# Nablax/Path-Tracer-CUDA-OpenGL

Hardware: AMD Instinct MI355X
Metric: Mray/s + ms/frame, bunny-in-Cornell 1920×1080 @1024spp, 1/2/4/8 MI355X (higher is better)
Workload: dtype f32

## Files before the change

path-tracer-cuda-opengl_amd/csrc/pt_device.hip:

```cpp
#include <hip/hip_runtime.h>

#include <algorithm>
#include <array>
#include <atomic>
#include <chrono>
#include <cfloat>
#include <cmath>
#include <cstdio>
#include <cstdlib>
#include <cstring>
#include <limits>
#include <type_traits>
#include <memory>
#include <string>
#include <vector>

#include "../host/pt_error.hpp"
#include "../host/pt_host.hpp"
#include "../host/pt_inst_dev.hpp"
#include "../host/pt_instancing.hpp"
#include "../host/pt_wide8.hpp"
#include "../host/pt_wide_dev.hpp"
#include "pt.h"
#include "pt_math.hpp"

using pt::fail;

#include "pt_prims.hpp"

namespace pt {
int launchCompatWide(int stack, const void* params, hipStream_t st);
int compatWideWavesPerCU(int stack, int& n);
}

#define HIP_TRY(expr)                                                                        \
    do {                                                                                     \
        hipError_t _e = (expr);                                                              \
        if (_e != hipSuccess)                                                                \
            return fail(PT_ERR_HIP, std::string(#expr) + ": " + hipGetErrorString(_e));      \
    } while (0)

namespace {

constexpr int kWave = 64;
constexpr uint32_t kLeafBit = 0x80000000u;
constexpr uint32_t kSphereBit = 0x40000000u;
constexpr uint32_t kPrimMask = 0x3fffffffu;
constexpr int kJumpMats = 32;
constexpr int kNumCounters = 32;

struct DevScene {
    const float4* nodes;
    const float4* prims;
    const float4* shade;
    const float4* mats;
// ... 293 lines not shown
    const float3 s1 = cross3(d, e2);
    const float det = dot3(s1, e1);
    const float3 s = sub(o, v0);
    const float3 s2 = cross3(s, e1);
    const float inv = rcpRNWave(det, hasM);
    const float t = dot3(s2, e2) * inv;
    const float b1 = dot3(s1, s) * inv;
    const float b2 = dot3(s2, d) * inv;
    const int k = (int)__float_as_uint(q.p0.w);
    const uint64_t rejM = __ballot(b1 >= 1.0f) | __ballot(b1 <= 0.0f) | __ballot(b2 >= 1.0f) | __ballot(b2 <= 0.0f) |
                          __ballot(b1 + b2 >= 1.0f);
    const uint64_t hitM = hasM & __ballot(det != 0.0f) & __ballot(t > tmin) & ~rejM;
    const uint64_t takeM = hitM & (__ballot(t < closest) | (__ballot(t == closest) & __ballot(k < best)));
    const float mid = __builtin_amdgcn_fmed3f(t, closest, t2);
    t2 = __builtin_amdgcn_inverse_ballot_w64(hitM) ? mid : t2;
    closest = __builtin_amdgcn_inverse_ballot_w64(takeM) ? t : closest;
    best = __builtin_amdgcn_inverse_ballot_w64(takeM) ? k : best;
}
__device__ __forceinline__ bool deferredRedo(float4 xy, float2 z, float3 o, float3 inv, float closest, float t2) {
    const SlabHit b = slabPair(v2f{xy.x, xy.y}, v2f{xy.z, xy.w}, v2f{z.x, z.y}, o, inv, 0.001f, __builtin_inff());
    return !b.hit || (closest < b.lo && t2 < b.lo);
}

template <bool MIX = false>
__device__ __forceinline__ uint32_t wideHits(uint4 n0, uint4 n1, uint4 n2, uint4 n3, uint4 n4, float3 o, float3 inv,
                                             uint32_t oct, float tmin, float tmax) {
    constexpr uint32_t kMixExp = MIX ? 24u : 0u;
    const float ax = __uint_as_float(((n0.w & 0xffu) + kMixExp) << 23) * inv.x;
    const float ay = __uint_as_float((((n0.w >> 8) & 0xffu) + kMixExp) << 23) * inv.y;
    const float az = __uint_as_float((((n0.w >> 16) & 0xffu) + kMixExp) << 23) * inv.z;
    const float bx = (__uint_as_float(n0.x) - o.x) * inv.x;
    const float by = (__uint_as_float(n0.y) - o.y) * inv.y;
    const float bz = (__uint_as_float(n0.z) - o.z) * inv.z;
    const bool sx = inv.x < 0.0f, sy = inv.y < 0.0f, sz = inv.z < 0.0f;
    const uint32_t nearX[2] = {sx ? n2.z : n2.x, sx ? n2.w : n2.y}, farX[2] = {sx ? n2.x : n2.z, sx ? n2.y : n2.w};
    const uint32_t nearY[2] = {sy ? n3.z : n3.x, sy ? n3.w : n3.y}, farY[2] = {sy ? n3.x : n3.z, sy ? n3.y : n3.w};
    const uint32_t nearZ[2] = {sz ? n4.z : n4.x, sz ? n4.w : n4.y}, farZ[2] = {sz ? n4.x : n4.z, sz ? n4.y : n4.w};
    uint32_t hits = 0u;
#pragma unroll
    for (int h = 0; h < 2; h++) {
        const uint32_t meta4 = h ? n1.w : n1.z;
        const uint32_t inner4 = __builtin_amdgcn_bitop3_b32(meta4, meta4 << 1, 0x10101010u, 0x80);
        const uint32_t inner1 = inner4 >> 4;
        const uint32_t bitIndex4 = (meta4 ^ mulHalves(inner1, oct)) & 0x1f1f1f1fu;
        uint32_t childBits4 = (meta4 >> 5) & 0x07070707u;
        asm("" : "+v"(childBits4));
#pragma unroll
        for (int j = 0; j < 4; j++) {
            float tnx, tny, tnz, tfx, tfy, tfz;
            if constexpr (MIX) {
                const bool hi = (j & 2) != 0;
                const uint32_t px = hi ? planePairHi(nearX[h]) : planePairLo(nearX[h]);
                const uint32_t py = hi ? planePairHi(nearY[h]) : planePairLo(nearY[h]);
// ... 467 lines not shown
    unsigned* taskCounter;
    uint32_t* stackSpill;
    uint32_t ntasks;
    int nwaves;
    uint32_t seed0, seed1;
    uint32_t sampleBase;
    int measureCost;
    int camFar;
    int rawOut;
    int stripeShift, blockShift;
    int splitTiles, splitWays;
    int compatGrid;
    int nCrit, critLanes, critWaves;
    const uint32_t* critList;
    const uint8_t* critFlag;
    uint32_t* pixRays;
    float3 skyH, skyZ;
    int lit;
    const float4* lights;
    int nLights;
    int mis;
    const uint32_t* lightSlot;
    const uint32_t* instLightFirst;
};
template <bool LIT>
__device__ __forceinline__ float3 skyOf(const RenderParams& P, float3 d, float3 att) {
    if constexpr (LIT) return sky(d, att, P.skyH, P.skyZ);
    else return sky(d, att);
}

#ifndef PT_CRIT_PIXELS
#define PT_CRIT_PIXELS 256
#endif
#ifndef PT_CRIT_LANES
#define PT_CRIT_LANES 4
#endif
constexpr int kCritPixels = PT_CRIT_PIXELS;
constexpr int kCritLanes = PT_CRIT_LANES;
__host__ __device__ constexpr bool critFor(bool sample, bool wide, bool inst, int stack) {
    return !sample && wide && !inst && stack <= 8;
}
__device__ __forceinline__ void addBlock(unsigned long long* acc, float3 sum, uint32_t rays, bool cost) {
    const bool small = sum.x >= 0.0f && sum.y >= 0.0f && sum.z >= 0.0f &&
                       fmaxf(fmaxf(sum.x, sum.y), sum.z) < 16777216.0f;
    unsigned long long fx, fy, fz;
    if (__ballot(!small) == 0) {
// ... 227 lines not shown
typedef const __attribute__((address_space(4))) uint32_t* KU32;
__device__ __forceinline__ float3 ld3(const __attribute__((address_space(4))) float3& v) {
    KFloat* f = (KFloat*)&v;
    return f3(f[0], f[1], f[2]);
}
__device__ __forceinline__ DevScene ldScene(KArgs k) {
    DevScene S;
    S.nodes = k->S.nodes; S.prims = k->S.prims; S.shade = k->S.shade; S.mats = k->S.mats;
    S.wnodes = k->S.wnodes; S.wprims = k->S.wprims; S.wshade = k->S.wshade; S.wbox = k->S.wbox; S.rankOf = k->S.rankOf;
    S.iparent = k->S.iparent; S.err = k->S.err; S.nprims = k->S.nprims;
    S.hasSpheres = k->S.hasSpheres;
    S.cx = k->S.cx; S.cy = k->S.cy; S.cz = k->S.cz; S.ext = k->S.ext;
    S.mixLim = k->S.mixLim;
    S.winst = k->S.winst; S.gBits = k->S.gBits;
    return S;
}

template <bool LIT>
__device__ __forceinline__ float3 skyK(float3 d, float3 att) {
    if constexpr (LIT) return sky(d, att, ld3(kargs()->skyH), ld3(kargs()->skyZ));
    else return sky(d, att);
}

template <int STACK, bool SAMPLE, bool WIDE, bool INST = false, bool LIT = false, bool NEE = false, bool MIS = false>
__global__ __launch_bounds__(kWave) __attribute__((amdgpu_waves_per_eu(kWavesPerEU<STACK, SAMPLE, WIDE> - (NEE && STACK >= 16 ? 1 : 0)))) void renderKernelWF(RenderParams P) {
    static_assert(!NEE || (WIDE && LIT), "NEE: the wide kernels' LIT instantiations only");
    static_assert(!MIS || NEE, "MIS: the NEE instantiations only");
    constexpr int LS = kLdsStack<STACK, SAMPLE, WIDE>;
    __shared__ uint32_t stk[LS * kWave];
    constexpr int SPECN = WIDE && !INST ? PT_WIDE_SPEC : 0;
    constexpr bool SPEC = SPECN > 0;
    __shared__ uint32_t pend[SPEC ? 2 * SPECN * kWave : 1];
    __shared__ float wray[INST ? 6 * kWave : 1];
    __shared__ uint4 taskState[SAMPLE ? kWave : 1];
    __shared__ float neeV[NEE ? (MIS ? 10 : 9) * kWave : 1];
    __shared__ uint32_t neeF[NEE ? kWave : 1];
    const int lane = threadIdx.x;
    int bidT = (int)blockIdx.x, slice = -1;
    constexpr bool CRITK = critFor(SAMPLE, WIDE, INST, STACK);
    const bool crit = CRITK && bidT < P.critWaves;
    if constexpr (CRITK) {
        if (!crit) bidT -= P.critWaves;
    }
    if constexpr (!SAMPLE) {
        const int ks = P.splitTiles * P.splitWays;
        if (crit) {
        } else if (bidT < ks) { slice = bidT % P.splitWays; bidT /= P.splitWays; }
        else bidT -= ks - P.splitTiles;
    }
    int tile = (SAMPLE || crit) ? -1 : tileOf(P, bidT), nSamples = SAMPLE ? 0 : P.spp;
// ... 63 lines not shown


#define PT_BEGIN_RAY(SH)                                                                            \
    do {                                                                                          \
        const bool sh_ = NEE && (SH);                                                             \
        if constexpr (NEE) depthLeft -= sh_ ? 0 : 1;                                              \
        else depthLeft--;                                                                         \
        if constexpr (SAMPLE) {    \
            if (kargs()->measureCost)                                                             \
                __hip_atomic_fetch_add(&taskState[lane].w, 1u, __ATOMIC_RELAXED, __HIP_MEMORY_SCOPE_WORKGROUP); \
        }                                                                                         \
        closest = sh_ ? kShadowTmax : __builtin_inff();                                           \
        best = -1;                                                                                \
        sp = 0;                                                                                   \
        qn = 0;                                                                                   \
        if constexpr (CRITK) pxRays++;                                                            \
        if constexpr (WIDE) {                 \
            inv = f3(rcpRN(d.x), rcpRN(d.y), rcpRN(d.z));                                         \
            const uint32_t oc_ = (inv.x < 0.0f ? 1u : 0u) | (inv.y < 0.0f ? 2u : 0u) | (inv.z < 0.0f ? 4u : 0u); \
            oct = oc_;                                                                            \
            tg = 0u;                                                                              \
                    \
                   \
            bestLo = INST || kargs()->S.hasSpheres ? -__builtin_inff() : closest;                  \
            ng = S.nprims > 0 ? (1u << oc_) : 0u;                                                 \
                 \
            if (!INST && ((kargs()->camFar && !sh_ && depthLeft + 1 == kargs()->max_depth) ||      \
                          (PT_WIDE_MIX && mixUnsafe(inv, kargs()->S.mixLim)))) {                   \
                ng = 0u;             \
                oct |= 8u;      \
            }                                                                                     \
            if (INST && kargs()->camFar && !sh_ && depthLeft + 1 == kargs()->max_depth) {          \
                     \
                const auto& K_ = *kargs();                                                        \
                (void)instEntry(K_.S.cx, K_.S.cy, K_.S.cz, K_.S.ext, o, d, inv);                   \
            }                                                                                     \
            if (CRITK && crit) PT_CRIT_TRACE();                                                    \
        } else if (S.nprims <= 1) {                                                               \
            node = -1;                                                                            \
            if (S.nprims == 1) {        \
                const float t1 = primHitT(loadPrim(S, 0), __float_as_uint(S.prims[2].w) != 0, o, d, \
                                          0.001f, closest);                                       \
                if (t1 >= 0.0f) { closest = t1; best = 0; }                                       \
            }                                                                                     \
        } else {                                                                                  \
            inv = f3(rcpRN(d.x), rcpRN(d.y), rcpRN(d.z));                                         \
            node = 0;                                                                             \
        }                                                                                         \
    } while (0)
#define PT_CRIT_TRACE()                                                                             \
    do {                                                                                          \
        const bool lb_ = S.nprims > 1;                                                            \
        const bool sph_ = kargs()->S.hasSpheres != 0;                                             \
        bool redo_ = false;                                                                       \
        for (;;) {                                                                                \
            while (tg) {                                                                          \
                const uint32_t k_ = tgBase + (uint32_t)__builtin_ctz(tg);                         \
                tg &= tg - 1u;                                                                    \
                const float4* w_ = reinterpret_cast<const float4*>(reinterpret_cast<const char*>(S.wprims) + mul48(k_)); \
                const Prim q_{w_[0], w_[1], w_[2]};                                               \
                const bool isS_ = __float_as_uint(q_.p2.w) != 0u;                                 \
                sTris += (uint32_t)__popcll(__ballot(!isS_));                                     \
                sSph += (uint32_t)__popcll(__ballot(isS_));                                       \
                if (sph_) wideTest<true>(q_, o, d, inv, 0.001f, closest, best, bestLo, lb_, redo_, 0u); \
                else if (INST) wideTest<false>(q_, o, d, inv, 0.001f, closest, best, bestLo, lb_, redo_, 0u); \
                else wideTestTri(q_, __ballot(true), o, d, 0.001f, closest, best, bestLo);    \
            }                                                                                     \
            if ((ng & 0xffu) == 0u) {                                                             \
                if (sp == 0) break;                                                               \
                sp--;                                                                             \
                ng = my[sp * kWave];                                                              \
            }                                                                                     \
            const uint32_t bit_ = (uint32_t)__builtin_ctz(ng & 0xffu);                            \
            const uint32_t child_ = (ng >> 8) + (bit_ ^ (oct & 7u));                              \
            ng &= ~(1u << bit_);                                                                  \
            if (ng & 0xffu) { my[sp * kWave] = ng; sp++; }    \
            sVisits += (uint32_t)__popcll(__ballot(true));                                        \
            const uint32_t off_ = mul80(child_);                                                  \
            const uint4 n0_ = __builtin_bit_cast(uint4, __builtin_amdgcn_raw_buffer_load_b128(nodeRsrc, off_, 0, 0)); \
            const uint4 n1_ = __builtin_bit_cast(uint4, __builtin_amdgcn_raw_buffer_load_b128(nodeRsrc, off_ + 16u, 0, 0)); \
            const uint4 n2_ = __builtin_bit_cast(uint4, __builtin_amdgcn_raw_buffer_load_b128(nodeRsrc, off_ + 32u, 0, 0)); \
            const uint4 n3_ = __builtin_bit_cast(uint4, __builtin_amdgcn_raw_buffer_load_b128(nodeRsrc, off_ + 48u, 0, 0)); \
            const uint4 n4_ = __builtin_bit_cast(uint4, __builtin_amdgcn_raw_buffer_load_b128(nodeRsrc, off_ + 64u, 0, 0)); \
            const uint32_t h_ = wideHits<PT_WIDE_MIX != 0>(n0_, n1_, n2_, n3_, n4_, o, inv, oct & 7u, 0.001f, closest); \
            ng = (n1_.x << 8) | (h_ >> 24);                                                      \
            tgBase = n1_.y;                                                                       \
            tg = h_ & 0xffffffu;                                                                  \
        }                                                                                         \
        if (redo_) oct |= 8u;              \
// ... 223 lines not shown
                        tg = hits & 0xffffffu;
                    }
                }
            } else if constexpr (WIDE) {
                if (wantNode) {
                    if (SPEC && laneOf(mL)) {
                        const uint32_t c = SPECN == 1 ? 0u : (oct >> 4) & 3u;
                        pend[(2u * c) * kWave + lane] = tgBase;
                        pend[(2u * c + 1u) * kWave + lane] = tg;
                        oct += 16u;
                    }
                    if constexpr (SPEC) asm volatile("" ::: "memory");
                    if ((ng & 0xffu) == 0u) { sp--; ng = my[sp * kWave]; }
                    const uint32_t bit = (uint32_t)__builtin_ctz(ng & 0xffu);
                    const uint32_t child = (ng >> 8) + (bit ^ (oct & 7u));
                    ng &= ~(1u << bit);
                    if (ng & 0xffu) { my[sp * kWave] = ng; sp++; }
                    const uint32_t off = mul80(child);
                    const uint4 n0 = __builtin_bit_cast(uint4, __builtin_amdgcn_raw_buffer_load_b128(nodeRsrc, off, 0, 0));
                    const uint4 n1 = __builtin_bit_cast(uint4, __builtin_amdgcn_raw_buffer_load_b128(nodeRsrc, off + 16u, 0, 0));
                    const uint4 n2 = __builtin_bit_cast(uint4, __builtin_amdgcn_raw_buffer_load_b128(nodeRsrc, off + 32u, 0, 0));
                    const uint4 n3 = __builtin_bit_cast(uint4, __builtin_amdgcn_raw_buffer_load_b128(nodeRsrc, off + 48u, 0, 0));
                    const uint4 n4 = __builtin_bit_cast(uint4, __builtin_amdgcn_raw_buffer_load_b128(nodeRsrc, off + 64u, 0, 0));
                    const uint32_t hits = wideHits<PT_WIDE_MIX != 0>(n0, n1, n2, n3, n4, o, inv, oct & 7u, 0.001f, closest);
                    ng = (n1.x << 8) | (hits >> 24);
                    tgBase = n1.y;
                    tg = hits & 0xffffffu;
#ifdef PT_DIAG
                    oct &= ~64u;
#endif
                    if (SPEC && tg == 0u && (oct & 48u)) {
                        oct -= 16u;
                        const uint32_t c = SPECN == 1 ? 0u : (oct >> 4) & 3u;
                        tgBase = pend[(2u * c) * kWave + lane];
                        tg = pend[(2u * c + 1u) * kWave + lane];
#ifdef PT_DIAG
                        oct |= 64u;
#endif
                    }
                }
            } else if (wantNode) {
                const uint32_t off = (uint32_t)node * 64u;
                const float4 a = bload4(nodeRsrc, off), b = bload4(nodeRsrc, off + 16u);
                const float4 q = bload4(nodeRsrc, off + 32u), r = bload4(nodeRsrc, off + 48u);
                const uint32_t lref = __float_as_uint(r.x), rref = __float_as_uint(r.y);
                SlabHit2 h2 = slabBoth(a, b, q, o, inv, 0.001f, closest);
                asm volatile("" : "+v"(h2.r.lo));
// ... 49 lines not shown
            if constexpr (WIDE) {
                PT_DIAG_ADD(sPops, (uint32_t)nL);
                uint32_t k0 = 0u, k1 = 0u;
                const bool h0 = laneOf(mL);
                if (h0) k0 = tgBase + (uint32_t)__builtin_ctz(tg);
                tg &= tg - 1u;
                const uint64_t m1 = __ballot((int)tg > 0);
                const bool h1 = laneOf(m1);
                if (h1) k1 = tgBase + (uint32_t)__builtin_ctz(tg);
                tg &= tg - 1u;
                const float4* w0 = reinterpret_cast<const float4*>(reinterpret_cast<const char*>(S.wprims) + mul48(k0));
                const float4* w1 = reinterpret_cast<const float4*>(reinterpret_cast<const char*>(S.wprims) + mul48(k1));
                const Prim q0{w0[0], w0[1], w0[2]}, q1{w1[0], w1[1], w1[2]};
                bool redo = false;
#ifdef PT_DIAG
                {
                    sHalf += (unsigned long long)__popcll(__ballot(h0 && !h1));
                    const bool pk = !INST && (oct & 64u) != 0u;
                    sParkT += (unsigned long long)(__popcll(__ballot(pk && h0)) + __popcll(__ballot(pk && h1)));
                }
#endif
                const bool lb = !INST && S.nprims > 1;
                const uint32_t kh = INST ? (oct >> 8) << kargs()->S.gBits : 0u;
                if (kargs()->S.hasSpheres) {
                    if (h0) wideTest<true>(q0, o, d, inv, 0.001f, closest, best, bestLo, lb, redo, kh);
                    if (h1) wideTest<true>(q1, o, d, inv, 0.001f, closest, best, bestLo, lb, redo, kh);
                    const uint64_t s0 = mL & __ballot(__float_as_uint(q0.p2.w) != 0u);
                    const uint64_t s1 = m1 & __ballot(__float_as_uint(q1.p2.w) != 0u);
                    sTris += (uint32_t)nL + (uint32_t)__popcll(m1) - (uint32_t)__popcll(s0) - (uint32_t)__popcll(s1);
                    sSph += (uint32_t)__popcll(s0) + (uint32_t)__popcll(s1);
                } else {
                    if constexpr (INST) {
                        if (h0) wideTest<false>(q0, o, d, inv, 0.001f, closest, best, bestLo, lb, redo, kh);
                        if (h1) wideTest<false>(q1, o, d, inv, 0.001f, closest, best, bestLo, lb, redo, kh);
                    } else {
                        wideTestTri(q0, mL, o, d, 0.001f, closest, best, bestLo);
                        wideTestTri(q1, m1, o, d, 0.001f, closest, best, bestLo);
                    }
                    sTris += (uint32_t)nL + (uint32_t)__popcll(m1);
                }
                if (redo) oct |= 8u;
                if (SPEC && tg == 0u && (oct & 48u)) {
                    oct -= 16u;
                    const uint32_t c = SPECN == 1 ? 0u : (oct >> 4) & 3u;
                    tgBase = pend[(2u * c) * kWave + lane];
                    tg = pend[(2u * c + 1u) * kWave + lane];
#ifdef PT_DIAG
// ... 24 lines not shown
                    {
                        tested = true;
                        const float t = primHitT(pr, sph, o, d, 0.001f, closest);
                        if (t >= 0.0f) { closest = t; best = (int)k; }
                    }
                }
            }
            sTris += (uint32_t)__popcll(__ballot(tested && !sph));
            sSph += (uint32_t)__popcll(__ballot(tested && sph));
            }
            }
        }
        if (kind == 2) {
            const uint64_t shadeM = mS & ~needTaskM;
            const bool shading = laneOf(shadeM);
            uint32_t nf = 0u;
            if constexpr (NEE) nf = neeF[lane];
            const bool shadowQ = NEE && (nf & 1u) != 0u;
            if constexpr (WIDE && !INST) {
                bool redo = shading && (oct & 8u);
#ifdef PT_DIAG
                bool missed = false;
#endif
                if (!kargs()->S.hasSpheres && S.nprims > 1) {
                    if (shading && best >= 0 && !redo) {
                        const float4* bx = kargs()->S.wbox + 2 * (size_t)best;
                        redo = deferredRedo(bx[0], *reinterpret_cast<const float2*>(bx + 1), o, inv, closest, bestLo);
#ifdef PT_DIAG
                        {
                            const float2 bz_ = *reinterpret_cast<const float2*>(bx + 1);
                            const float4 bx_ = bx[0];
                            missed = !slabPair(v2f{bx_.x, bx_.y}, v2f{bx_.z, bx_.w}, v2f{bz_.x, bz_.y}, o, inv, 0.001f,
                                               __builtin_inff()).hit;
                        }
#endif
                    }
                }
                PT_DIAG_ADD(sRedo, (uint32_t)__popcll(__ballot(redo)));
                PT_DIAG_ADD(sRedoMiss, (uint32_t)__popcll(__ballot(missed)));
                if (redo) {
                    const DevScene S2 = ldScene(kargs());
                    closest = shadowQ ? kShadowTmax : __builtin_inff();
                    const int k = traceRefStackless(S2, o, d, 0.001f, closest);
                    best = k >= 0 ? (int)S2.rankOf[k] : -1;
                }
            }
            PT_DIAG_ADD(itS, 1u);
// ... 154 lines not shown
        atomicAdd(P.counters + 18, cycNp);
        atomicAdd(P.counters + 19, cycBr);
        atomicAdd(P.counters + 20, (unsigned long long)sRedo);
        atomicAdd(P.counters + 21, sSpecN);
        atomicAdd(P.counters + 22, sIdleN);
        atomicAdd(P.counters + 23, (unsigned long long)sRedoMiss);
        atomicAdd(P.counters + 25, sHalf);
        atomicAdd(P.counters + 27, sParkT);
#endif
    }
}
#undef PT_BEGIN_RAY
#undef PT_CRIT_TRACE
#undef PT_NEW_PATH
#undef PT_SKY
#undef PT_TAKE_TASKS
#undef PT_FINISH_TASK
#undef PT_DIAG_ADD

#ifdef PT_TU_COMPAT
}

namespace pt {
int launchCompatWide(int stack, const void* params, hipStream_t st) {
    const RenderParams& P = *static_cast<const RenderParams*>(params);
    const int grid = P.compatGrid;
    switch (stack) {
#define PT_COMPAT_WIDE(S)                                                                    \
        case S:                                                                                  \
            if (P.nLights > 0 && P.mis) renderKernelWF<S, false, true, false, true, true, true><<<grid, kWave, 0, st>>>(P); \
            else if (P.nLights > 0) renderKernelWF<S, false, true, false, true, true><<<grid, kWave, 0, st>>>(P); \
            else if (P.lit) renderKernelWF<S, false, true, false, true><<<grid, kWave, 0, st>>>(P); \
            else renderKernelWF<S, false, true><<<grid, kWave, 0, st>>>(P);                      \
            break;
        PT_COMPAT_WIDE(8)
        PT_COMPAT_WIDE(16)
        PT_COMPAT_WIDE(24)
#undef PT_COMPAT_WIDE
        default: return -1;
    }
    return 0;
}
int compatWideWavesPerCU(int stack, int& n) {
    const void* k = stack == 8 ? reinterpret_cast<const void*>(&renderKernelWF<8, false, true>)
                  : stack == 16 ? reinterpret_cast<const void*>(&renderKernelWF<16, false, true>)
                  : stack == 24 ? reinterpret_cast<const void*>(&renderKernelWF<24, false, true>) : nullptr;
    if (!k || hipOccupancyMaxActiveBlocksPerMultiprocessor(&n, k, kWave, 0) != hipSuccess) return -1;
    return 0;
}
}
#else

__global__ __launch_bounds__(256) void resolveKernel(const float* __restrict__ src,
                                                     const unsigned long long* __restrict__ pixAcc, float* accum,
                                                     float inv, int format, void* out, int64_t npix,
                                                     unsigned* tileCost, int width, int tilesX, int costMax) {
    const int64_t i = (int64_t)blockIdx.x * blockDim.x + threadIdx.x;
    if (i >= npix) return;
    float x, y, z;
    if (!pixAcc) {
        x = src[3 * i + 0]; y = src[3 * i + 1]; z = src[3 * i + 2];
    } else {
        const ulonglong2* a2 = reinterpret_cast<const ulonglong2*>(pixAcc + 4 * i);
        const ulonglong2 a = a2[0], b = a2[1];
        x = fixedToFloat(a.x);
        y = fixedToFloat(a.y);
        z = fixedToFloat(b.x);
        const uint32_t rays = (uint32_t)min(b.y, 0xffffffffull);
        if (tileCost) {
// ... 1275 lines not shown
    s->wideDepth = topDepth + 1 + s->instMaxDepthB + 1;
    s->wideSource = 4;
    s->wideReady = true;
    s->instLights = lights;
    s->nLights = lights ? s->instLightTotal : 0;
    s->buildMs = (double)ms;
    s->wideBuildMs = std::chrono::duration<double, std::milli>(std::chrono::steady_clock::now() - t0).count();
    s->depth = 0;
    if (wideStackFor(s->wideDepth) < 0) return fail(PT_ERR_STATE, "instanced BVH too deep");
    s->built = true;
    *done = true;
    return PT_OK;
}

int setDevice(int dev) {
    int count = 0;
    if (hipGetDeviceCount(&count) != hipSuccess || count <= 0)
        return fail(PT_ERR_NODEVICE, "no HIP device visible (the library has no CPU fallback)");
    if (dev < 0 || dev >= count) return fail(PT_ERR_INVALID, "device index out of range");
    HIP_TRY(hipSetDevice(dev));
    return PT_OK;
}

template <int S, bool LIT>
void launchRenderWide(const RenderParams& P, hipStream_t st) {
    if (P.S.winst) {
        if constexpr (LIT) {
            if (P.nLights > 0) {
                if (P.pixAcc && P.mis) renderKernelWF<S, true, true, true, true, true, true><<<P.nwaves, kWave, 0, st>>>(P);
                else if (P.pixAcc) renderKernelWF<S, true, true, true, true, true><<<P.nwaves, kWave, 0, st>>>(P);
                else if (P.mis) renderKernelWF<S, false, true, true, true, true, true><<<P.compatGrid, kWave, 0, st>>>(P);
                else renderKernelWF<S, false, true, true, true, true><<<P.compatGrid, kWave, 0, st>>>(P);
                return;
            }
        }
        if (P.pixAcc) renderKernelWF<S, true, true, true, LIT><<<P.nwaves, kWave, 0, st>>>(P);
        else renderKernelWF<S, false, true, true, LIT><<<P.compatGrid, kWave, 0, st>>>(P);
        return;
    }
    if (P.pixAcc) {
        if constexpr (LIT) {
            if (P.nLights > 0) {
                if (P.mis) renderKernelWF<S, true, true, false, true, true, true><<<P.nwaves, kWave, 0, st>>>(P);
                else renderKernelWF<S, true, true, false, true, true><<<P.nwaves, kWave, 0, st>>>(P);
                return;
            }
        }
        renderKernelWF<S, true, true, false, LIT><<<P.nwaves, kWave, 0, st>>>(P);
    } else {
        pt::launchCompatWide(S, &P, st);
    }
}
template <int S, bool LIT>
void launchRender(const RenderParams& P, hipStream_t st) {
    if (P.kernel == PT_KERNEL_WAVEFRONT && P.pixAcc)
        renderKernelWF<S, true, false, false, LIT><<<P.nwaves, kWave, 0, st>>>(P);
    else if (P.kernel == PT_KERNEL_WAVEFRONT)
        renderKernelWF<S, false, false, false, LIT><<<P.compatGrid, kWave, 0, st>>>(P);
    else if (LIT && P.nLights > 0 && P.mis && P.pixAcc) renderKernel<S, true, LIT, LIT, LIT><<<P.ntiles, kWave, 0, st>>>(P);
    else if (LIT && P.nLights > 0 && P.mis) renderKernel<S, false, LIT, LIT, LIT><<<P.ntiles, kWave, 0, st>>>(P);
    else if (LIT && P.nLights > 0 && P.pixAcc) renderKernel<S, true, LIT, LIT><<<P.ntiles, kWave, 0, st>>>(P);
    else if (LIT && P.nLights > 0) renderKernel<S, false, LIT, LIT><<<P.ntiles, kWave, 0, st>>>(P);
    else if (P.pixAcc) renderKernel<S, true, LIT><<<P.ntiles, kWave, 0, st>>>(P);
    else renderKernel<S, false, LIT><<<P.ntiles, kWave, 0, st>>>(P);
}
template <int S, bool WIDE, bool INST = false, bool SAMPLE = true>
int wavesPerCU(int& n) {
    HIP_TRY(hipOccupancyMaxActiveBlocksPerMultiprocessor(&n, reinterpret_cast<const void*>(&renderKernelWF<S, SAMPLE, WIDE, INST>),
                                                         kWave, 0));
    return PT_OK;
}
template <int... Ns, class F>
bool withStack(int stack, F f) {
    return ((stack == Ns && (f(std::integral_constant<int, Ns>{}), true)) || ...);
}
template <class F>
bool withWideStack(int stack, F f) { return withStack<8, 16, 24>(stack, f); }
template <class F>
bool withBinStack(int stack, F f) { return withStack<16, 24, 32, 48, 64, 80>(stack, f); }

int persistentWavesPerCU(int stack, int kernel, int& n, bool inst, bool sample, bool nee, bool mis) {
    const bool wide = kernel == PT_KERNEL_WIDE;
    if (wide && sample && nee) {
        int rc = PT_OK;
        const bool ok = withWideStack(stack, [&](auto N) {
            constexpr int K = decltype(N)::value;
            const void* k = inst ? (mis ? reinterpret_cast<const void*>(&renderKernelWF<K, true, true, true, true, true, true>)
                                        : reinterpret_cast<const void*>(&renderKernelWF<K, true, true, true, true, true>))
                                 : (mis ? reinterpret_cast<const void*>(&renderKernelWF<K, true, true, false, true, true, true>)
                                        : reinterpret_cast<const void*>(&renderKernelWF<K, true, true, false, true, true>));
            const hipError_t e = hipOccupancyMaxActiveBlocksPerMultiprocessor(&n, k, kWave, 0);
            if (e != hipSuccess) rc = fail(PT_ERR_HIP, std::string("hipOccupancyMaxActiveBlocksPerMultiprocessor: ") + hipGetErrorString(e));
        });
        if (!ok) return fail(PT_ERR_STATE, "unsupported wide BVH depth");
        return rc;
    }
    if (wide && !inst && !sample)
        return pt::compatWideWavesPerCU(stack, n) ? fail(PT_ERR_STATE, "unsupported wide BVH depth") : PT_OK;
    int rc = PT_OK;
    const bool ok = wide ? withWideStack(stack, [&](auto N) {
        constexpr int K = decltype(N)::value;
        rc = !inst ? wavesPerCU<K, true>(n) : sample ? wavesPerCU<K, true, true>(n) : wavesPerCU<K, true, true, false>(n);
    }) : withBinStack(stack, [&](auto N) {
        constexpr int K = decltype(N)::value;
        rc = sample ? wavesPerCU<K, false>(n) : wavesPerCU<K, false, false, false>(n);
    });
    if (!ok) return fail(PT_ERR_STATE, !wide ? "unsupported BVH depth" : inst ? "unsupported instanced BVH depth" : "unsupported wide BVH depth");
    return rc;
}
int dispatchRender(int stack, const RenderParams& P, hipStream_t st) {
    const bool wide = P.kernel == PT_KERNEL_WIDE;
    const bool ok = wide ? withWideStack(stack, [&](auto N) {
        constexpr int K = decltype(N)::value;
        P.lit ? launchRenderWide<K, true>(P, st) : launchRenderWide<K, false>(P, st);
    }) : withBinStack(stack, [&](auto N) {
        constexpr int K = decltype(N)::value;
        P.lit ? launchRender<K, true>(P, st) : launchRender<K, false>(P, st);
    });
    if (!ok) return fail(PT_ERR_STATE, wide ? "unsupported wide BVH depth" : "unsupported BVH depth");
    HIP_TRY(hipGetLastError());
    return PT_OK;
}

unsigned queryBlocks(int64_t n) {
    int dev = 0, cus = 256;
// ... 783 lines not shown
    const bool nee = neeFlag && s->nLights > 0;
    const bool mis = misFlag && nee;
    const int rng = opts ? opts->rng : PT_RNG_COMPAT;
    if (rng != PT_RNG_COMPAT && rng != PT_RNG_SAMPLE) return fail(PT_ERR_INVALID, "pt_render_ex: unknown rng mode");
    if (kernel == PT_KERNEL_WIDE && (rc = ensureWide(s))) return rc;

    if (!f->ev0) {
        HIP_TRY(hipEventCreate(&f->ev0));
        HIP_TRY(hipEventCreate(&f->ev1));
        HIP_TRY(hipEventCreateWithFlags(&f->ev2, hipEventDisableTiming));
    }
    if (!f->counters.p && (rc = devAlloc(f->counters, kNumCounters * sizeof(unsigned long long)))) return rc;
    if (!f->hostCounters) HIP_TRY(hipHostMalloc(reinterpret_cast<void**>(&f->hostCounters),
                                                kNumCounters * sizeof(unsigned long long), hipHostMallocDefault));
    void* dst = out;
    if (!on_dev) {
        if ((rc = devReserve(f->staging, (size_t)std::max<int64_t>(1, np) * outBpp))) return rc;
        dst = f->staging.p;
    }
    HIP_TRY(hipMemsetAsync(f->counters.p, 0, kNumCounters * sizeof(unsigned long long), st));
    RenderParams P;
    P.S = devScene(s);
    P.S.err = reinterpret_cast<unsigned int*>(f->counters.as<unsigned long long>() + 7);
    if (s->wideReady && s->haveWtris && !s->hasSpheres && !s->instanced) P.S.wprims = s->wtris.as<float4>();
    P.cam.pos = make_float3(cam->origin[0], cam->origin[1], cam->origin[2]);
    P.cam.ll = make_float3(cam->lower_left[0], cam->lower_left[1], cam->lower_left[2]);
    P.cam.hor = make_float3(cam->horizontal[0], cam->horizontal[1], cam->horizontal[2]);
    P.cam.ver = make_float3(cam->vertical[0], cam->vertical[1], cam->vertical[2]);
    P.cam.right = make_float3(cam->right[0], cam->right[1], cam->right[2]);
    P.cam.up = make_float3(cam->up[0], cam->up[1], cam->up[2]);
    P.cam.lens = cam->lens_radius;
    P.skyH = make_float3(s->skyH[0], s->skyH[1], s->skyH[2]);
    P.skyZ = make_float3(s->skyZ[0], s->skyZ[1], s->skyZ[2]);
    {
        static const float H0[3] = {1.0f, 1.0f, 1.0f}, Z0[3] = {0.5f, 0.7f, 1.0f};
        P.lit = (s->hasEmissive || std::memcmp(s->skyH, H0, sizeof(H0)) != 0 || std::memcmp(s->skyZ, Z0, sizeof(Z0)) != 0) ? 1 : 0;
    }
    P.lights = nee ? s->lights.as<float4>() : nullptr;
    P.nLights = nee ? (int)s->nLights : 0;
    P.mis = mis ? 1 : 0;
    P.lightSlot = mis ? s->lightSlot.as<uint32_t>() : nullptr;
    P.instLightFirst = mis && s->instanced ? s->instLightFirst.as<uint32_t>() : nullptr;
    uint32_t* b = f->state.as<uint32_t>();
    P.sd = b; P.s0 = b + np; P.s1 = b + 2 * np; P.s2 = b + 3 * np; P.s3 = b + 4 * np; P.s4 = b + 5 * np;
    P.out = static_cast<float*>(dst);
    P.rawOut = 0;
    P.sampleBase = 0;
// ... 43 lines not shown
    P.leafBatch = (opts && opts->leaf_batch > 0) ? std::min(opts->leaf_batch, 64)
                                                 : envInt("PT_LEAF_BATCH", instWide ? 16 : (wideSample || wideFlatCompat) ? wideBatch
                                                                                                       : (sampleRng ? 24 : 20));
    P.nodeMin = std::getenv("PT_NODE_MIN") ? std::atoi(std::getenv("PT_NODE_MIN")) : 8;
    P.shadeBatch = (opts && opts->shade_batch > 0) ? std::min(opts->shade_batch, 64)
                                                   : envInt("PT_SHADE_BATCH", instWide ? 20 : (wideSample || wideFlatCompat) ? wideBatch
                                                                                                           : (sampleRng ? 32 : 12));
    if (kernel == PT_KERNEL_SIMPLE) P.leafBatch = 0;
    const size_t ntl = (size_t)std::max(1, P.ntiles);
    if (!f->tileCost.p) {
        if ((rc = devAlloc(f->tileCost, ntl * 4)) || (rc = devAlloc(f->tileOrder, ntl * 4)) ||
            (rc = devAlloc(f->tileXY, ntl * 4)) || (rc = devAlloc(f->tileXYId, ntl * 4)))
            return rc;
        f->haveOrder = false;
    }
    const bool lpt = !(opts && (opts->flags & PT_RENDER_IDENTITY_ORDER));
    const bool sample = rng == PT_RNG_SAMPLE && np > 0 && P.ntiles > 0;
    if (!f->cus) {
        if (hipDeviceGetAttribute(&f->cus, hipDeviceAttributeMultiprocessorCount, f->device) != hipSuccess)
            f->cus = 256;
        f->cus = std::max(f->cus, 1);
    }
    auto perCUFor = [&](int& perCU) -> int {
        static std::atomic<int> cached[16][2][2][2][3][3];
        const bool small = stack <= 24 && stack % 8 == 0 && f->device >= 0 && f->device < 16;
        std::atomic<int>* c = small ? &cached[f->device][sample ? 1 : 0][s->instanced ? 1 : 0]
                                             [kernel == PT_KERNEL_WIDE ? 1 : 0][stack / 8 - 1][mis ? 2 : nee ? 1 : 0] : nullptr;
        const int known = c ? c->load(std::memory_order_relaxed) : 0;
        if (known > 0) {
            perCU = known;
            return PT_OK;
        }
        if (int r = persistentWavesPerCU(stack, kernel, perCU, s->instanced, sample, nee, mis)) return r;
        if (c) c->store(perCU, std::memory_order_relaxed);
        return PT_OK;
    };
    P.nCrit = 0;
    P.critLanes = std::max(1, std::min(64, envCount("PT_CRIT_LANES", kCritLanes)));
    P.critWaves = 0;
    P.critList = nullptr;
    P.critFlag = nullptr;
    P.pixRays = nullptr;
    const bool critOn = lpt && !nee && critFor(sample, kernel == PT_KERNEL_WIDE, s->instanced, stack) && np > 0 &&
                        max_depth > 16 && envCount("PT_CRIT_PIXELS", kCritPixels) > 0;
    if (critOn) {
        if ((rc = devReserve(f->pixRays, (size_t)np * 4))) return rc;
        P.pixRays = f->pixRays.as<uint32_t>();
        if (f->critK > 0) {
            P.nCrit = f->critK;
            P.critWaves = (P.nCrit + P.critLanes - 1) / P.critLanes;
            P.critList = f->pixSorted.as<uint32_t>();
            P.critFlag = f->critFlag.as<uint8_t>();
        }
    }
    P.splitWays = std::max(1, std::min(8, envCount("PT_SPLIT_WAYS", 2)));
    P.splitTiles = (lpt && f->haveOrder && !sample && kernel != PT_KERNEL_SIMPLE)
// ... 194 lines not shown
```

Baseline: 22680.

## Specialize flat wide kernels for triangle-only scenes via TRI template

Adds a TRI template parameter to the wide render kernel. It is chosen at launch when the scene has only triangle records and no instancing, and defaults to on. In that specialization the runtime sphere checks and mixed sphere/triangle test paths are removed at compile time and triangles are tested directly. For the sample kernel, child-box exponent decoding also switches to explicit bitfield-extract instructions. This removes branches and likely register pressure, but adds more kernel instantiations and uses separate occupancy queries.

Result: faster. 23150, median of 6 (+2.1%).

```diff
diff --git a/path-tracer-cuda-opengl_amd/csrc/pt_device.hip b/path-tracer-cuda-opengl_amd/csrc/pt_device.hip
--- a/path-tracer-cuda-opengl_amd/csrc/pt_device.hip
+++ b/path-tracer-cuda-opengl_amd/csrc/pt_device.hip
@@ -30,7 +30,7 @@
 
 namespace pt {
 int launchCompatWide(int stack, const void* params, hipStream_t st);
-int compatWideWavesPerCU(int stack, int& n);
+int compatWideWavesPerCU(int stack, bool tri, int& n);
 }
 
 #define HIP_TRY(expr)                                                                        \
@@ -370,13 +370,24 @@
     return !b.hit || (closest < b.lo && t2 < b.lo);
 }
 
-template <bool MIX = false>
+template <bool MIX = false, bool DEC3 = false>
 __device__ __forceinline__ uint32_t wideHits(uint4 n0, uint4 n1, uint4 n2, uint4 n3, uint4 n4, float3 o, float3 inv,
                                              uint32_t oct, float tmin, float tmax) {
     constexpr uint32_t kMixExp = MIX ? 24u : 0u;
-    const float ax = __uint_as_float(((n0.w & 0xffu) + kMixExp) << 23) * inv.x;
-    const float ay = __uint_as_float((((n0.w >> 8) & 0xffu) + kMixExp) << 23) * inv.y;
-    const float az = __uint_as_float((((n0.w >> 16) & 0xffu) + kMixExp) << 23) * inv.z;
+    float ax, ay, az;
+    if constexpr (DEC3) {
+        uint32_t ex, ey, ez;
+        asm("v_bfe_u32 %0, %1, 0, 8" : "=v"(ex) : "v"(n0.w));
+        asm("v_bfe_u32 %0, %1, 8, 8" : "=v"(ey) : "v"(n0.w));
+        asm("v_bfe_u32 %0, %1, 16, 8" : "=v"(ez) : "v"(n0.w));
+        ax = __uint_as_float((ex << 23) + (kMixExp << 23)) * inv.x;
+        ay = __uint_as_float((ey << 23) + (kMixExp << 23)) * inv.y;
+        az = __uint_as_float((ez << 23) + (kMixExp << 23)) * inv.z;
+    } else {
+        ax = __uint_as_float(((n0.w & 0xffu) + kMixExp) << 23) * inv.x;
+        ay = __uint_as_float((((n0.w >> 8) & 0xffu) + kMixExp) << 23) * inv.y;
+        az = __uint_as_float((((n0.w >> 16) & 0xffu) + kMixExp) << 23) * inv.z;
+    }
     const float bx = (__uint_as_float(n0.x) - o.x) * inv.x;
     const float by = (__uint_as_float(n0.y) - o.y) * inv.y;
     const float bz = (__uint_as_float(n0.z) - o.z) * inv.z;
@@ -890,6 +901,7 @@
     int mis;
     const uint32_t* lightSlot;
     const uint32_t* instLightFirst;
+    int tri;
 };
 template <bool LIT>
 __device__ __forceinline__ float3 skyOf(const RenderParams& P, float3 d, float3 att) {
@@ -1163,10 +1175,12 @@
     else return sky(d, att);
 }
 
-template <int STACK, bool SAMPLE, bool WIDE, bool INST = false, bool LIT = false, bool NEE = false, bool MIS = false>
+template <int STACK, bool SAMPLE, bool WIDE, bool INST = false, bool LIT = false, bool NEE = false, bool MIS = false,
+          bool TRI = false>
 __global__ __launch_bounds__(kWave) __attribute__((amdgpu_waves_per_eu(kWavesPerEU<STACK, SAMPLE, WIDE> - (NEE && STACK >= 16 ? 1 : 0)))) void renderKernelWF(RenderParams P) {
     static_assert(!NEE || (WIDE && LIT), "NEE: the wide kernels' LIT instantiations only");
     static_assert(!MIS || NEE, "MIS: the NEE instantiations only");
+    static_assert(!TRI || (WIDE && !INST), "TRI: the flat wide kernels only");
     constexpr int LS = kLdsStack<STACK, SAMPLE, WIDE>;
     __shared__ uint32_t stk[LS * kWave];
     constexpr int SPECN = WIDE && !INST ? PT_WIDE_SPEC : 0;
@@ -1276,7 +1290,8 @@
             tg = 0u;                                                                              \
                     \
                    \
-            bestLo = INST || kargs()->S.hasSpheres ? -__builtin_inff() : closest;                  \
+            if constexpr (TRI) bestLo = closest;                                                  \
+            else bestLo = INST || kargs()->S.hasSpheres ? -__builtin_inff() : closest;            \
             ng = S.nprims > 0 ? (1u << oc_) : 0u;                                                 \
                  \
             if (!INST && ((kargs()->camFar && !sh_ && depthLeft + 1 == kargs()->max_depth) ||      \
@@ -1305,7 +1320,8 @@
 #define PT_CRIT_TRACE()                                                                             \
     do {                                                                                          \
         const bool lb_ = S.nprims > 1;                                                            \
-        const bool sph_ = kargs()->S.hasSpheres != 0;                                             \
+        bool sph_ = false;                                                                        \
+        if constexpr (!TRI) sph_ = kargs()->S.hasSpheres != 0;                                    \
         bool redo_ = false;                                                                       \
         for (;;) {                                                                                \
             while (tg) {                                                                          \
@@ -1313,12 +1329,17 @@
                 tg &= tg - 1u;                                                                    \
                 const float4* w_ = reinterpret_cast<const float4*>(reinterpret_cast<const char*>(S.wprims) + mul48(k_)); \
                 const Prim q_{w_[0], w_[1], w_[2]};                                               \
+                if constexpr (TRI) {                                 \
+                    sTris += (uint32_t)__popcll(__ballot(true));                                  \
+                    wideTestTri(q_, __ballot(true), o, d, 0.001f, closest, best, bestLo);         \
+                } else {                                                                          \
                 const bool isS_ = __float_as_uint(q_.p2.w) != 0u;                                 \
                 sTris += (uint32_t)__popcll(__ballot(!isS_));                                     \
                 sSph += (uint32_t)__popcll(__ballot(isS_));                                       \
                 if (sph_) wideTest<true>(q_, o, d, inv, 0.001f, closest, best, bestLo, lb_, redo_, 0u); \
                 else if (INST) wideTest<false>(q_, o, d, inv, 0.001f, closest, best, bestLo, lb_, redo_, 0u); \
                 else wideTestTri(q_, __ballot(true), o, d, 0.001f, closest, best, bestLo);    \
+                }                                                                                 \
             }                                                                                     \
             if ((ng & 0xffu) == 0u) {                                                             \
                 if (sp == 0) break;                                                               \
@@ -1588,7 +1609,7 @@
                     const uint4 n2 = __builtin_bit_cast(uint4, __builtin_amdgcn_raw_buffer_load_b128(nodeRsrc, off + 32u, 0, 0));
                     const uint4 n3 = __builtin_bit_cast(uint4, __builtin_amdgcn_raw_buffer_load_b128(nodeRsrc, off + 48u, 0, 0));
                     const uint4 n4 = __builtin_bit_cast(uint4, __builtin_amdgcn_raw_buffer_load_b128(nodeRsrc, off + 64u, 0, 0));
-                    const uint32_t hits = wideHits<PT_WIDE_MIX != 0>(n0, n1, n2, n3, n4, o, inv, oct & 7u, 0.001f, closest);
+                    const uint32_t hits = wideHits<PT_WIDE_MIX != 0, TRI && SAMPLE>(n0, n1, n2, n3, n4, o, inv, oct & 7u, 0.001f, closest);
                     ng = (n1.x << 8) | (hits >> 24);
                     tgBase = n1.y;
                     tg = hits & 0xffffffu;
@@ -1684,7 +1705,11 @@
 #endif
                 const bool lb = !INST && S.nprims > 1;
                 const uint32_t kh = INST ? (oct >> 8) << kargs()->S.gBits : 0u;
-                if (kargs()->S.hasSpheres) {
+                if constexpr (TRI) {
+                    wideTestTri(q0, mL, o, d, 0.001f, closest, best, bestLo);
+                    wideTestTri(q1, m1, o, d, 0.001f, closest, best, bestLo);
+                    sTris += (uint32_t)nL + (uint32_t)__popcll(m1);
+                } else if (kargs()->S.hasSpheres) {
                     if (h0) wideTest<true>(q0, o, d, inv, 0.001f, closest, best, bestLo, lb, redo, kh);
                     if (h1) wideTest<true>(q1, o, d, inv, 0.001f, closest, best, bestLo, lb, redo, kh);
                     const uint64_t s0 = mL & __ballot(__float_as_uint(q0.p2.w) != 0u);
@@ -1755,7 +1780,9 @@
 #ifdef PT_DIAG
                 bool missed = false;
 #endif
-                if (!kargs()->S.hasSpheres && S.nprims > 1) {
+                bool triScene = TRI;
+                if constexpr (!TRI) triScene = !kargs()->S.hasSpheres;
+                if (triScene && S.nprims > 1) {
                     if (shading && best >= 0 && !redo) {
                         const float4* bx = kargs()->S.wbox + 2 * (size_t)best;
                         redo = deferredRedo(bx[0], *reinterpret_cast<const float2*>(bx + 1), o, inv, closest, bestLo);
@@ -1956,16 +1983,20 @@
 }
 
 namespace pt {
+template <int S, bool TRI>
+static void launchCompatWideTri(const RenderParams& P, hipStream_t st) {
+    const int grid = P.compatGrid;
+    if (P.nLights > 0 && P.mis) renderKernelWF<S, false, true, false, true, true, true, TRI><<<grid, kWave, 0, st>>>(P);
+    else if (P.nLights > 0) renderKernelWF<S, false, true, false, true, true, false, TRI><<<grid, kWave, 0, st>>>(P);
+    else if (P.lit) renderKernelWF<S, false, true, false, true, false, false, TRI><<<grid, kWave, 0, st>>>(P);
+    else renderKernelWF<S, false, true, false, false, false, false, TRI><<<grid, kWave, 0, st>>>(P);
+}
 int launchCompatWide(int stack, const void* params, hipStream_t st) {
     const RenderParams& P = *static_cast<const RenderParams*>(params);
-    const int grid = P.compatGrid;
     switch (stack) {
 #define PT_COMPAT_WIDE(S)                                                                    \
         case S:                                                                                  \
-            if (P.nLights > 0 && P.mis) renderKernelWF<S, false, true, false, true, true, true><<<grid, kWave, 0, st>>>(P); \
-            else if (P.nLights > 0) renderKernelWF<S, false, true, false, true, true><<<grid, kWave, 0, st>>>(P); \
-            else if (P.lit) renderKernelWF<S, false, true, false, true><<<grid, kWave, 0, st>>>(P); \
-            else renderKernelWF<S, false, true><<<grid, kWave, 0, st>>>(P);                      \
+            P.tri ? launchCompatWideTri<S, true>(P, st) : launchCompatWideTri<S, false>(P, st);   \
             break;
         PT_COMPAT_WIDE(8)
         PT_COMPAT_WIDE(16)
@@ -1975,10 +2006,14 @@
     }
     return 0;
 }
-int compatWideWavesPerCU(int stack, int& n) {
-    const void* k = stack == 8 ? reinterpret_cast<const void*>(&renderKernelWF<8, false, true>)
-                  : stack == 16 ? reinterpret_cast<const void*>(&renderKernelWF<16, false, true>)
-                  : stack == 24 ? reinterpret_cast<const void*>(&renderKernelWF<24, false, true>) : nullptr;
+template <bool TRI>
+static const void* compatWideKernel(int stack) {
+    return stack == 8 ? reinterpret_cast<const void*>(&renderKernelWF<8, false, true, false, false, false, false, TRI>)
+         : stack == 16 ? reinterpret_cast<const void*>(&renderKernelWF<16, false, true, false, false, false, false, TRI>)
+         : stack == 24 ? reinterpret_cast<const void*>(&renderKernelWF<24, false, true, false, false, false, false, TRI>) : nullptr;
+}
+int compatWideWavesPerCU(int stack, bool tri, int& n) {
+    const void* k = tri ? compatWideKernel<true>(stack) : compatWideKernel<false>(stack);
     if (!k || hipOccupancyMaxActiveBlocksPerMultiprocessor(&n, k, kWave, 0) != hipSuccess) return -1;
     return 0;
 }
@@ -3300,6 +3335,17 @@
     return PT_OK;
 }
 
+template <int S, bool LIT, bool TRI>
+void launchSampleWideFlat(const RenderParams& P, hipStream_t st) {
+    if constexpr (LIT) {
+        if (P.nLights > 0) {
+            if (P.mis) renderKernelWF<S, true, true, false, true, true, true, TRI><<<P.nwaves, kWave, 0, st>>>(P);
+            else renderKernelWF<S, true, true, false, true, true, false, TRI><<<P.nwaves, kWave, 0, st>>>(P);
+            return;
+        }
+    }
+    renderKernelWF<S, true, true, false, LIT, false, false, TRI><<<P.nwaves, kWave, 0, st>>>(P);
+}
 template <int S, bool LIT>
 void launchRenderWide(const RenderParams& P, hipStream_t st) {
     if (P.S.winst) {
@@ -3317,14 +3363,7 @@
         return;
     }
     if (P.pixAcc) {
-        if constexpr (LIT) {
-            if (P.nLights > 0) {
-                if (P.mis) renderKernelWF<S, true, true, false, true, true, true><<<P.nwaves, kWave, 0, st>>>(P);
-                else renderKernelWF<S, true, true, false, true, true><<<P.nwaves, kWave, 0, st>>>(P);
-                return;
-            }
-        }
-        renderKernelWF<S, true, true, false, LIT><<<P.nwaves, kWave, 0, st>>>(P);
+        P.tri ? launchSampleWideFlat<S, LIT, true>(P, st) : launchSampleWideFlat<S, LIT, false>(P, st);
     } else {
         pt::launchCompatWide(S, &P, st);
     }
@@ -3342,10 +3381,10 @@
     else if (P.pixAcc) renderKernel<S, true, LIT><<<P.ntiles, kWave, 0, st>>>(P);
     else renderKernel<S, false, LIT><<<P.ntiles, kWave, 0, st>>>(P);
 }
-template <int S, bool WIDE, bool INST = false, bool SAMPLE = true>
+template <int S, bool WIDE, bool INST = false, bool SAMPLE = true, bool TRI = false>
 int wavesPerCU(int& n) {
-    HIP_TRY(hipOccupancyMaxActiveBlocksPerMultiprocessor(&n, reinterpret_cast<const void*>(&renderKernelWF<S, SAMPLE, WIDE, INST>),
-                                                         kWave, 0));
+    HIP_TRY(hipOccupancyMaxActiveBlocksPerMultiprocessor(
+        &n, reinterpret_cast<const void*>(&renderKernelWF<S, SAMPLE, WIDE, INST, false, false, false, TRI>), kWave, 0));
     return PT_OK;
 }
 template <int... Ns, class F>
@@ -3357,7 +3396,7 @@
 template <class F>
 bool withBinStack(int stack, F f) { return withStack<16, 24, 32, 48, 64, 80>(stack, f); }
 
-int persistentWavesPerCU(int stack, int kernel, int& n, bool inst, bool sample, bool nee, bool mis) {
+int persistentWavesPerCU(int stack, int kernel, int& n, bool inst, bool sample, bool nee, bool mis, bool tri) {
     const bool wide = kernel == PT_KERNEL_WIDE;
     if (wide && sample && nee) {
         int rc = PT_OK;
@@ -3365,6 +3404,8 @@
             constexpr int K = decltype(N)::value;
             const void* k = inst ? (mis ? reinterpret_cast<const void*>(&renderKernelWF<K, true, true, true, true, true, true>)
                                         : reinterpret_cast<const void*>(&renderKernelWF<K, true, true, true, true, true>))
+                          : tri  ? (mis ? reinterpret_cast<const void*>(&renderKernelWF<K, true, true, false, true, true, true, true>)
+                                        : reinterpret_cast<const void*>(&renderKernelWF<K, true, true, false, true, true, false, true>))
                                  : (mis ? reinterpret_cast<const void*>(&renderKernelWF<K, true, true, false, true, true, true>)
                                         : reinterpret_cast<const void*>(&renderKernelWF<K, true, true, false, true, true>));
             const hipError_t e = hipOccupancyMaxActiveBlocksPerMultiprocessor(&n, k, kWave, 0);
@@ -3374,11 +3415,11 @@
         return rc;
     }
     if (wide && !inst && !sample)
-        return pt::compatWideWavesPerCU(stack, n) ? fail(PT_ERR_STATE, "unsupported wide BVH depth") : PT_OK;
+        return pt::compatWideWavesPerCU(stack, tri, n) ? fail(PT_ERR_STATE, "unsupported wide BVH depth") : PT_OK;
     int rc = PT_OK;
     const bool ok = wide ? withWideStack(stack, [&](auto N) {
         constexpr int K = decltype(N)::value;
-        rc = !inst ? wavesPerCU<K, true>(n) : sample ? wavesPerCU<K, true, true>(n) : wavesPerCU<K, true, true, false>(n);
+        rc = !inst ? (tri ? wavesPerCU<K, true, false, true, true>(n) : wavesPerCU<K, true>(n)) : sample ? wavesPerCU<K, true, true>(n) : wavesPerCU<K, true, true, false>(n);
     }) : withBinStack(stack, [&](auto N) {
         constexpr int K = decltype(N)::value;
         rc = sample ? wavesPerCU<K, false>(n) : wavesPerCU<K, false, false, false>(n);
@@ -4208,7 +4249,9 @@
     RenderParams P;
     P.S = devScene(s);
     P.S.err = reinterpret_cast<unsigned int*>(f->counters.as<unsigned long long>() + 7);
-    if (s->wideReady && s->haveWtris && !s->hasSpheres && !s->instanced) P.S.wprims = s->wtris.as<float4>();
+    const bool triRecords = s->wideReady && s->haveWtris && !s->hasSpheres && !s->instanced;
+    if (triRecords) P.S.wprims = s->wtris.as<float4>();
+    P.tri = triRecords && kernel == PT_KERNEL_WIDE && envCount("PT_WIDE_TRI", 1) != 0 ? 1 : 0;
     P.cam.pos = make_float3(cam->origin[0], cam->origin[1], cam->origin[2]);
     P.cam.ll = make_float3(cam->lower_left[0], cam->lower_left[1], cam->lower_left[2]);
     P.cam.hor = make_float3(cam->horizontal[0], cam->horizontal[1], cam->horizontal[2]);
@@ -4298,16 +4341,16 @@
         f->cus = std::max(f->cus, 1);
     }
     auto perCUFor = [&](int& perCU) -> int {
-        static std::atomic<int> cached[16][2][2][2][3][3];
+        static std::atomic<int> cached[16][2][2][2][3][3][2];
         const bool small = stack <= 24 && stack % 8 == 0 && f->device >= 0 && f->device < 16;
         std::atomic<int>* c = small ? &cached[f->device][sample ? 1 : 0][s->instanced ? 1 : 0]
-                                             [kernel == PT_KERNEL_WIDE ? 1 : 0][stack / 8 - 1][mis ? 2 : nee ? 1 : 0] : nullptr;
+                                             [kernel == PT_KERNEL_WIDE ? 1 : 0][stack / 8 - 1][mis ? 2 : nee ? 1 : 0][P.tri] : nullptr;
         const int known = c ? c->load(std::memory_order_relaxed) : 0;
         if (known > 0) {
             perCU = known;
             return PT_OK;
         }
-        if (int r = persistentWavesPerCU(stack, kernel, perCU, s->instanced, sample, nee, mis)) return r;
+        if (int r = persistentWavesPerCU(stack, kernel, perCU, s->instanced, sample, nee, mis, P.tri != 0)) return r;
         if (c) c->store(perCU, std::memory_order_relaxed);
         return PT_OK;
     };
```
